# deemoe404/rmcv

Measured on AMD Instinct MI355X. Metric: frames/sec (1280x1024 BGR) armour detect, higher is better.
Workload: dtype u8

## Files before the change

rmcv_amd/csrc/contours_device.h:

```cpp
#pragma once
#include <stddef.h>
#include <stdlib.h>
#include <string.h>

#include "rmcv_internal.h"
#include "wave_detect.h"

namespace rmcv {

__device__ __forceinline__ uint64_t ld_l2(const uint64_t* p)
{
    return __hip_atomic_load(p, __ATOMIC_RELAXED, __HIP_MEMORY_SCOPE_AGENT);
}
__device__ __forceinline__ unsigned long long ld_l2(const unsigned long long* p)
{
    return __hip_atomic_load(p, __ATOMIC_RELAXED, __HIP_MEMORY_SCOPE_AGENT);
}

__device__ __forceinline__ uint64_t win_load(const uint32_t* plane32, int prow, int y, int xb)
{
    const uint32_t* p = plane32 + ((int64_t)(y + 1) * prow + 1) * 2 + (xb >> 5);
    uint64_t v;
    __builtin_memcpy(&v, p, 8);
    return v;
// ... 135 lines not shown
            const int L = __ffsll((long long)m) - 1;
            const int x0 = __shfl(found, L), y0 = band * 64 + L;
            if (lane < L) done = true;
            int len = 0, ymax = y0;
            if (lane == 0) {
                const int room = (nc < max_contours && np < max_points) ? (max_points - np) : 0;
                len = trace_border(t, x0, y0, pts + np, room, &ymax);
                if (nc < max_contours) { cs[nc] = np; cl[nc] = len; }
                __builtin_amdgcn_fence(__ATOMIC_RELEASE, "workgroup");
            }
            len = __shfl(len, 0);
            ymax = __shfl(ymax, 0);
            if (nc >= max_contours) st |= RMCV_FRAME_OVF_CONTOURS;
            if (np + len > max_points) { st |= RMCV_FRAME_OVF_POINTS; }
            nc++;
            np = (np + len > max_points) ? max_points : np + len;
            if (lane == L) { xmin = x0 + 1; dirty = true; }
            else if (lane > L && y <= ymax) dirty = true;
        }
    }
    *nc_out = nc < max_contours ? nc : max_contours;
    *np_out = np;
    *st_out = st;
}

__device__ __forceinline__ int dir_dx(int s) { return (s == 0 || s == 1 || s == 7) ? 1 : ((s >= 3 && s <= 5) ? -1 : 0); }
__device__ __forceinline__ int dir_dy(int s) { return (s >= 1 && s <= 3) ? -1 : ((s >= 5) ? 1 : 0); }

struct LabelStore {
    const uint32_t* rowmask;
    const uint16_t* rowbase;
    unsigned long long* lab;
    unsigned long long* neg;
    __device__ __forceinline__ int slot(int y, int k) const { return rowbase[y] + __popc(rowmask[y] & ((1u << k) - 1u)); }
};

#ifndef RMCV_KEPT_CAP
#define RMCV_KEPT_CAP 512
#endif
static constexpr int KEPT_CAP = RMCV_KEPT_CAP;
#ifndef RMCV_SLOT_CAP
#define RMCV_SLOT_CAP 1664
#endif
static constexpr int SLOT_CAP = RMCV_SLOT_CAP;
#ifndef RMCV_CT_THREADS_MAX
#define RMCV_CT_THREADS_MAX 512
#endif
static constexpr int CT_THREADS_MAX = RMCV_CT_THREADS_MAX;
static constexpr int MULTI_CAP = 32;
#ifndef RMCV_NN_CAP
#define RMCV_NN_CAP VISIT_CAP
#endif
static constexpr int NN_CAP = RMCV_NN_CAP;
static_assert(NN_CAP <= VISIT_CAP, "the visits' global scratch (Bufs::visit_xy) is VISIT_CAP entries per frame");
#ifndef RMCV_MID_PAD
#define RMCV_MID_PAD 0
#endif
#ifndef RMCV_CT_MAXH
#define RMCV_CT_MAXH 2048
#endif
static constexpr int CT_MAXH = RMCV_CT_MAXH;

struct ContoursLds {
    unsigned long long lab[SLOT_CAP], neg[SLOT_CAP];
    uint16_t nbase[SLOT_CAP], spos[SLOT_CAP];
    uint32_t kkey[KEPT_CAP];
    int32_t koff[KEPT_CAP], klen[KEPT_CAP];
    uint8_t kacc[KEPT_CAP];
    uint32_t multi[MULTI_CAP];
#if RMCV_MID_PAD > 0
    unsigned long long mid_pad[RMCV_MID_PAD / 8];
#endif
    int scan[CT_THREADS_MAX];
    uint32_t ringtab[256];
    uint32_t w_off[KEPT_CAP], w_cnt[KEPT_CAP];
    uint16_t n_a[NN_CAP], n_b[NN_CAP], n_d[NN_CAP];
    int nnodes, nkept, cursor, flags, nrows, nslots, nelig, lit[3];
    int nmulti;
    int revoked;
    int wnext;
    int sink[64];
};
static_assert(offsetof(ContoursLds, scan) >= (CT_THREADS_MAX / 64) * 3840, "the fused tail's wave-private rows (sizeof(WaveLds) = 3840 each) overlay dead tables only");
static_assert(offsetof(ContoursLds, scan) % 8 == 0 && offsetof(ContoursLds, w_off) % 8 == 0, "alignment");
static constexpr int MID_LDS_WORDS = (int)(offsetof(ContoursLds, scan) / 4);

struct RowTabs {
    uint32_t* rowmask;
    uint16_t* rows;
    uint16_t* rowbase;
};
__host__ __device__ static inline int lds_rows_cap(int h) { const int r = (h + 63) & ~63; return r < CT_MAXH ? r : CT_MAXH; }
__host__ __device__ static inline size_t lds_bytes(int h) { return sizeof(ContoursLds) + (size_t)lds_rows_cap(h) * 8; }
__device__ __forceinline__ RowTabs row_tabs(void* smem, int rows_cap)
{
    RowTabs R;
    R.rowmask = reinterpret_cast<uint32_t*>(reinterpret_cast<unsigned char*>(smem) + sizeof(ContoursLds));
    R.rows = reinterpret_cast<uint16_t*>(R.rowmask + rows_cap);
    R.rowbase = R.rows + rows_cap;
    return R;
}

constexpr uint32_t ring_entry(int ring)
{
    uint32_t backs[4] = {0, 0, 0, 0}, nexts[4] = {0, 0, 0, 0}, negs[4] = {0, 0, 0, 0};
    int cnt = 0, west0 = 0;
    if (ring == 0) {
        cnt = 1;
        west0 = 1;
        negs[0] = 1;
    } else {
        int wa = -1;
        for (int b = 0; b < 8; b++) {
            if (!((ring >> b) & 1)) continue;
            int d = (b + 1) & 7, axis = 0, west = 0, len = 0;
            while (!((ring >> d) & 1)) {
                axis |= !(d & 1);
                west |= d == 4;
                d = (d + 1) & 7;
                len++;
            }
            if (!len || !axis) continue;
            if (cnt < 4) {
                backs[cnt] = (uint32_t)b;
                nexts[cnt] = (uint32_t)d;
                negs[cnt] = ((unsigned)(d - 1) < (unsigned)b) ? 1u : 0u;
                if (west) wa = cnt;
            }
            cnt++;
        }
        if (wa > 0 && wa < 4) {
            uint32_t t = backs[0]; backs[0] = backs[wa]; backs[wa] = t;
            t = nexts[0]; nexts[0] = nexts[wa]; nexts[wa] = t;
            t = negs[0]; negs[0] = negs[wa]; negs[wa] = t;
        }
        west0 = wa >= 0;
    }
    uint32_t e = (uint32_t)(cnt > 7 ? 7 : cnt);
    for (int a = 0; a < 4; a++) e |= (backs[a] << (3 + 3 * a)) | (nexts[a] << (15 + 3 * a)) | (negs[a] << (28 + a));
    e |= (uint32_t)west0 << 27;
    return e;
}
struct RingTab {
    uint32_t v[256];
    constexpr RingTab() : v()
    {
        for (int r = 0; r < 256; r++) v[r] = ring_entry(r);
    }
};
static __device__ const RingTab RINGTAB = RingTab();

__device__ __forceinline__ uint32_t ring_of(int b, uint64_t ul, uint64_t uc, uint64_t ur, uint64_t ml, uint64_t mc, uint64_t mr,
                                            uint64_t dl, uint64_t dc, uint64_t dr)
{
    auto three = [&](uint64_t l, uint64_t c, uint64_t r) -> uint32_t {
        if (b == 0) return (uint32_t)(l >> 63) | ((uint32_t)(c & 3ull) << 1);
        if (b == 63) return (uint32_t)(c >> 62) | ((uint32_t)(r & 1ull) << 2);
        return (uint32_t)(c >> (b - 1)) & 7u;
    };
    const uint32_t u = three(ul, uc, ur), m = three(ml, mc, mr), d = three(dl, dc, dr);
    return ((m >> 2) & 1u) | (((u >> 2) & 1u) << 1) | (((u >> 1) & 1u) << 2) | ((u & 1u) << 3) | ((m & 1u) << 4) | ((d & 1u) << 5) |
           (((d >> 1) & 1u) << 6) | (((d >> 2) & 1u) << 7);
}

__device__ __forceinline__ void visit_masks(uint64_t ul, uint64_t uc, uint64_t ur, uint64_t ml, uint64_t mc, uint64_t mr, uint64_t dl,
                                            uint64_t dc, uint64_t dr, uint64_t* B, uint64_t* E2, uint64_t* E3, uint64_t* E4)
// ... 1055 lines not shown
```

rmcv_amd/csrc/k_contours_kernel.inc:

```
#define CT_THREADS KC_THREADS
#ifndef RMCV_KC_ATTR
#define RMCV_KC_ATTR
#endif
__global__ __launch_bounds__(CT_THREADS) RMCV_KC_ATTR void KC_KERNEL(const uint64_t* __restrict__ bits, const uint32_t* __restrict__ rowmasks,
                                                        int rm_pitch, uint64_t* lab, uint64_t* neg, int w, int h, int ww, int prow,
                                                        int64_t plane_pitch, rmcv_point* points, int32_t* cont_start,
                                                        int32_t* cont_len, int32_t* n_contours, int32_t* n_points,
                                                        int32_t* status, int max_contours, int max_points, int force_literal,
                                                        int32_t* __restrict__ elig, int32_t* __restrict__ n_elig,
                                                        int32_t* __restrict__ slot_kind, SparseTail X, uint32_t* __restrict__ visit_xy,
                                                        uint8_t* __restrict__ mid_base, int64_t mid_stride, int mid_slot_cap, SparseSched Q, int rows_cap)
{
    extern __shared__ unsigned long long smem_raw[];
#ifndef RMCV_KC_PRIO
#define RMCV_KC_PRIO 3
#endif
    __builtin_amdgcn_s_setprio(RMCV_KC_PRIO);
    ContoursLds& S = *reinterpret_cast<ContoursLds*>(smem_raw);
    const RowTabs RT = row_tabs(smem_raw, rows_cap);
    const int tid = threadIdx.x, lane = tid & 63, wave = tid >> 6;
    enum { FL_COMPLEX = 1, FL_MID = 2 };
    const int f = Q.order ? Q.order[blockIdx.x] : (int)blockIdx.x;
#ifdef RMCV_PROFILE_HANDOVER
    const long long th0_ = wall_clock64(), th1_ = th0_;
// ... 153 lines not shown
        if (tid == 0) S.flags = FL_COMPLEX;
        __syncthreads();
    }
    const bool literal = (S.flags & FL_COMPLEX) != 0;
    const bool complex = S.flags != 0;

    if (complex) {
        if (literal) {
        if (wave == 0) {
            int nc, np, st;
            literal_frame(lane, F, LAB, NEG, h, ww, prow, pts, cs, cl, max_contours, max_points,
                          summarised ? RT.rowmask : nullptr, &nc, &np, &st);
            if (lane == 0) { S.lit[0] = nc; S.lit[1] = np; S.lit[2] = st | RMCV_FRAME_SLOW_PATH; }
        }
        __threadfence();
        __syncthreads();
        for (int y = tid; y < h; y += CT_THREADS) {
            const int64_t base = (int64_t)(y + 1) * prow + 1;
            const uint32_t occ = summarised ? RT.rowmask[y] : ~0u;
            for (int k = 0; k < ww; k++)
                if ((k >= 32 || ((occ >> k) & 1u)) && F[base + k]) { LAB[base + k] = 0; NEG[base + k] = 0; }
        }
        }
        {
            const int nc = S.lit[0];
            int32_t* el = elig + (int64_t)f * max_contours;
            for (int k = tid; k < nc; k += CT_THREADS) {
                if (cl[k] >= 6) el[atomicAdd(&S.nelig, 1)] = k;
                else slot_kind[(int64_t)f * max_contours + (nc - 1 - k)] = 0;
            }
        }
        __syncthreads();
        if (tid == 0) {
            n_contours[f] = S.lit[0];
            n_points[f] = S.lit[1];
            n_elig[f] = S.nelig;
            status[f] = S.lit[2];
        }
    } else {
    STAMP();
#ifdef RMCV_PROFILE
    if (tid == 0 && (f == 0 || f == 100))
        printf("[f%d] rows=%d slots=%d nodes=%d kept=%d pts=%d | tables %.1f cycles %.1f V %.1f us\n", f, nrows, S.nslots, S.nnodes,
               nkept, S.cursor, (t_[1] - t_[0]) / 100.0, (t_[2] - t_[1]) / 100.0, (t_[3] - t_[2]) / 100.0);
#endif
    for (int e = tid; e < nkept; e += CT_THREADS) {
        const uint32_t key = S.kkey[e];
        int rank = 0;
        for (int j = 0; j < nkept; j++) rank += S.kkey[j] < key;
        cs[rank] = S.koff[e];
        cl[rank] = S.klen[e];
        if (S.klen[e] >= 6) {
            const int pos = atomicAdd(&S.nelig, 1);
            elig[(int64_t)f * max_contours + pos] = rank;
            S.n_d[pos] = (uint16_t)rank;
            S.w_off[pos] = (uint32_t)S.koff[e];
            S.w_cnt[pos] = (uint32_t)S.klen[e];
        } else slot_kind[(int64_t)f * max_contours + (nkept - 1 - rank)] = 0;
    }
    __syncthreads();
    if (tid == 0) {
        n_contours[f] = nkept;
        n_points[f] = S.cursor;
        n_elig[f] = S.nelig;
        status[f] = 0;
    }
    }
#if defined(RMCV_PROFILE) || defined(RMCV_PROFILE_HANDOVER)
    const long long tt0_ = wall_clock64();
#endif
    if (!X.fused) return;
    __syncthreads();
    const int nc = complex ? S.lit[0] : S.nkept;
    const int ne_all = S.nelig;
    const int ne_cap = !complex ? NN_CAP : (nc > 65535 ? 0 : 1024);
    const int ne = ne_all > ne_cap ? ne_cap : ne_all;
    const int32_t* el = elig + (int64_t)f * max_contours;
    uint16_t* const w_len = S.n_b;
    uint16_t* const w_idx = S.n_d;
    uint16_t* const w_sorted = S.n_a;
    const uint32_t* const w_off = S.w_off;
    const uint32_t* const w_cnt = S.w_cnt;
    static_assert(KEPT_CAP <= NN_CAP, "the work list fits the node tables");
    for (int e = tid; e < ne; e += CT_THREADS) {
        int len;
        if (complex) {
            const int k = el[e];
            len = cl[k];
            w_idx[e] = (uint16_t)k;
        } else len = (int)w_cnt[e];
        w_len[e] = (uint16_t)(len > 65535 ? 65535 : len);
    }
    if (tid == 0) S.wnext = 0;
    __syncthreads();
    for (int e = tid; e < ne; e += CT_THREADS) {
        const int len = w_len[e];
        int rank = 0;
        for (int j = 0; j < ne; j++) rank += (w_len[j] > len) || (w_len[j] == len && j < e);
        w_sorted[rank] = (uint16_t)e;
    }
    __syncthreads();
    {
        static_assert(offsetof(ContoursLds, n_a) >= (CT_THREADS_MAX / 64) * sizeof(WaveLds), "the work list must outlive the tables");
        static_assert(offsetof(ContoursLds, w_off) >= (CT_THREADS_MAX / 64) * sizeof(WaveLds), "... and so must its LDS copies of starts / lengths");
        WaveLds& L = reinterpret_cast<WaveLds*>(smem_raw)[wave];
        for (;;) {
            const int got = atomicAdd(lane == 0 ? &S.wnext : &S.sink[lane], lane == 0 ? 1 : 0);
            const int e = __shfl(got, 0);
            if (e >= ne_all) break;
            if (!complex) {
                const int pos = w_sorted[e];
                fit_contour_slot_at(f, (int)w_idx[pos], nc, pts, (int)w_off[pos], (int)w_cnt[pos], max_contours, max_points, X.G, slot_kind,
                                    X.slot_ell, L, lane);
            } else {
                const int k = e < ne ? (int)w_idx[w_sorted[e]] : el[e];
                fit_contour_slot(f, k, nc, pts, cs, cl, max_contours, max_points, X.G, slot_kind, X.slot_ell, L, lane);
            }
        }
    }
    __syncthreads();
#if defined(RMCV_PROFILE) || defined(RMCV_PROFILE_HANDOVER)
    const long long tt1_ = wall_clock64();
#endif
    if (wave == 0) {
        const FitTail& T = X.T;
        const int enemy = tail_enemy(T, f);
        const int np = blob_compact_frame(f, lane, slot_kind, X.slot_ell, nc, max_contours, enemy, T.blobs, T.blob_src, T.ellipses,
                                          T.neg_idx, T.n_blobs, T.n_neg, T.status, T.max_blobs);
        if (T.do_pairs) {
            __threadfence_block();
            armours_frame(f, lane, T.blobs, np, T.max_blobs, T.angle_diff_max, T.shear_max, T.length_ratio_max, enemy, T.armours,
                          T.n_armours, T.status, T.max_armours, T.ov);
        }
    }
#ifdef RMCV_PROFILE
    __syncthreads();
    if (tid == 0 && blockIdx.x < 2) printf("[tail b%d] eligible %d of %d contours: fits %.1f us, compaction + pairing %.1f us\n", (int)blockIdx.x, ne_all, nc, (tt1_ - tt0_) / 100.0, (wall_clock64() - tt1_) / 100.0);
#endif
#ifdef RMCV_PROFILE_HANDOVER
    __syncthreads();
    if (tid == 0)
        printf("[sp] %d %lld %lld %lld | %.1f %.1f %.1f %.1f %.1f | elig %d\n", f, th0_, th1_, (long long)wall_clock64(), (t_[1] - t_[0]) / 100.0,
               (t_[2] - t_[1]) / 100.0, (tt0_ - t_[2]) / 100.0, (tt1_ - tt0_) / 100.0, (wall_clock64() - tt1_) / 100.0, ne_all);
#endif
#ifndef KC_NO_CLASSIFY
    if (X.C.enabled) {
        __threadfence_block();
        __syncthreads();
        constexpr int NW = CT_THREADS / 64;
        static_assert((CT_THREADS_MAX / 64) * sizeof(WaveLds) + NW * (NFEAT * sizeof(float) + 32 * sizeof(double)) <= sizeof(ContoursLds), "feature rows fit");
        unsigned char* base = reinterpret_cast<unsigned char*>(smem_raw) + (CT_THREADS_MAX / 64) * sizeof(WaveLds);
        double* sums = reinterpret_cast<double*>(base) + wave * 32;
        float* feat = reinterpret_cast<float*>(base + NW * 32 * sizeof(double)) + wave * NFEAT;
        int na = X.T.n_armours[f];
        if (na > X.T.max_armours) na = X.T.max_armours;
        classify_frame(f, lane, wave, NW, na, X.C, X.T.armours, X.T.max_armours, feat, sums);
    }
#endif
}

#undef CT_THREADS
```

rmcv_amd/csrc/k_detect.hip:

```cpp
#include "device_hull.h"
#include "wave_detect.h"

namespace rmcv {

static constexpr int FIT_CHUNKS = 4;
__global__ __launch_bounds__(256) void k_fit(const rmcv_point* __restrict__ points, const int32_t* __restrict__ cont_start,
                                            const int32_t* __restrict__ cont_len, const int32_t* __restrict__ n_contours,
                                            int max_contours, int max_points, float tilt_max, float ratio_lo, float ratio_hi,
                                            double area_lo, double area_hi, int32_t* __restrict__ slot_kind,
                                            rmcv_rrect* __restrict__ slot_ell, const int32_t* __restrict__ elig,
                                            const int32_t* __restrict__ n_elig, int ov)
{
    __shared__ WaveLds lds[4];
    __builtin_amdgcn_s_setprio(3);
    const int f = blockIdx.x, lane = threadIdx.x & 63, wave = threadIdx.x >> 6;
    WaveLds& L = lds[wave];
    const int n = n_contours[f];
    const rmcv_point* pts = points + (int64_t)f * max_points;
    const int32_t* cs = cont_start + (int64_t)f * max_contours;
    const int32_t* cl = cont_len + (int64_t)f * max_contours;
    const int ne = n_elig[f];
    const FitGates G = {tilt_max, ratio_lo, ratio_hi, area_lo, area_hi, ov};
    for (int e = blockIdx.y * 4 + wave; e < ne; e += 4 * gridDim.y)
        fit_contour_slot(f, elig[(int64_t)f * max_contours + e], n, pts, cs, cl, max_contours, max_points, G, slot_kind, slot_ell, L, lane);
}

struct MatchArgs {
    float min_ratio, max_ratio, tilt_angle, min_area, max_area;
    int fit_ellipse, mode;
    int ov;
    int wcap, hcap, ccap;
    int pass;
    const uint8_t* frames;
    int64_t frame_pitch;
    int stride;
    const rmcv_point* win_eff;
};

static constexpr int MATCH_CHUNKS = 16;
static constexpr int MATCH_DEFERRED = 0x100;
__global__ __launch_bounds__(64) void k_match(const rmcv_point* __restrict__ points, const int32_t* __restrict__ cont_start,
                                             const int32_t* __restrict__ cont_len, const int32_t* __restrict__ n_contours,
                                             int max_contours, int max_points, MatchArgs A, int32_t* __restrict__ slot_kind,
                                             rmcv_rrect* __restrict__ slot_ell, const int32_t* __restrict__ elig,
                                             const int32_t* __restrict__ n_elig, int32_t* __restrict__ status)
{
    extern __shared__ unsigned long long match_smem[];
    __builtin_amdgcn_s_setprio(3);
    const int f = blockIdx.x, lane = threadIdx.x;
    WaveLds& L = *reinterpret_cast<WaveLds*>(match_smem);
    HullLds H;
    hull_lds_carve(reinterpret_cast<unsigned char*>(match_smem) + sizeof(WaveLds), A.wcap, A.hcap, A.ccap, H);
    const bool final_pass = A.pass == 1 || A.mode == 1;
    const int n = n_contours[f];
    const rmcv_point* pts = points + (int64_t)f * max_points;
    const int32_t* cs = cont_start + (int64_t)f * max_contours;
    const int32_t* cl = cont_len + (int64_t)f * max_contours;
    const int ne = A.mode == 1 ? n : n_elig[f];
    for (int e = blockIdx.y; e < ne; e += gridDim.y) {
        const int k = A.mode == 1 ? e : elig[(int64_t)f * max_contours + e];
        const int c = n - 1 - k;
        const int start = cs[k], len = cl[k];
        if (A.pass == 1 && slot_kind[(int64_t)f * max_contours + c] != MATCH_DEFERRED) continue;
        int word = 0;
        rmcv_rrect box = {0, 0, 0, 0, 0};
        if (len >= 1 && start + len <= max_points && (A.mode == 1 || len >= 6)) {
            const rmcv_point* cp = pts + start;
            double a00 = 0;
            long long sx = 0, sy = 0;
            int minx = INT_MAX, maxx = INT_MIN, miny = INT_MAX, maxy = INT_MIN;
            for (int i = lane; i < len; i += 64) {
                const rmcv_point p = cp[i], q = cp[i == 0 ? len - 1 : i - 1];
                a00 += (double)(float)q.x * (float)p.y - (double)(float)q.y * (float)p.x;
                sx += p.x;
                sy += p.y;
                minx = p.x < minx ? p.x : minx;
                maxx = p.x > maxx ? p.x : maxx;
                miny = p.y < miny ? p.y : miny;
                maxy = p.y > maxy ? p.y : maxy;
            }
            a00 = wave_sum_f64(a00);
            sx = wave_sum_i64(sx);
            sy = wave_sum_i64(sy);
            for (int d = 32; d >= 1; d >>= 1) {
                const int a = __shfl_xor(minx, d), b = __shfl_xor(maxx, d), cc = __shfl_xor(miny, d), dd = __shfl_xor(maxy, d);
                minx = a < minx ? a : minx;
                maxx = b > maxx ? b : maxx;
                miny = cc < miny ? cc : miny;
                maxy = dd > maxy ? dd : maxy;
            }
            const int W = maxx - minx + 1, Hh = maxy - miny + 1;
            const double area = dabs(a00 * 0.5);
            int ovf = 0;
            if (minx < 0 || miny < 0 || W > A.wcap || maxy >= HULL_MAX_DIM || len > (1 << 20)) ovf = 1;
            if (A.mode == 1) {
                if (!ovf) min_area_rect_wave(cp, len, minx, W, H, lane, &box, &ovf);
                word = 1;
                if (ovf && lane == 0) atomicOr(&status[f], RMCV_FRAME_HULL);
            } else if (!(area < A.min_area || area > A.max_area)) {
                rmcv_rrect ellipse;
                fit_ellipse_wave(cp, len, sx, sy, L, lane, &ellipse);
                if (A.fit_ellipse) {
                    box = ellipse;
                    ovf = 0;
                } else if (!ovf) {
                    min_area_rect_wave(cp, len, minx, W, H, lane, &box, &ovf);
                }
                if (ovf) {
                    word = final_pass ? 0 : MATCH_DEFERRED;
                    if (final_pass && lane == 0) atomicOr(&status[f], RMCV_FRAME_HULL);
                } else {
                    const float mx = box.w > box.h ? box.w : box.h, mn = box.w < box.h ? box.w : box.h;
                    const float ratio = mx / mn;
                    bool ok = !(ratio > A.max_ratio || ratio < A.min_ratio);
                    const float angle = ellipse.angle > 90 ? ellipse.angle - 90 : ellipse.angle + 90;
                    if (abs_ov(angle - 90, A.ov) > A.tilt_angle) ok = false;
                    if (ok) {
                        int camp = RMCV_CAMP_NEUTRAL;
                        if (A.frames)
                            camp = camp_from_mean_wave(A.frames + (int64_t)f * A.frame_pitch + frame_origin_offset(A.win_eff, f, A.stride), A.stride, minx, miny, W, Hh, lane);
                        word = 1 | ((camp + 2) << 4);
                    }
                }
            }
        }
        if (lane == 0) {
            slot_kind[(int64_t)f * max_contours + c] = word;
            slot_ell[(int64_t)f * max_contours + c] = box;
        }
    }
}


__global__ __launch_bounds__(64) void k_armours(const rmcv_lightblob* __restrict__ blobs, const int32_t* __restrict__ n_blobs,
                                               int max_blobs, float angle_diff_max, float shear_max,
                                               float length_ratio_max, int enemy, rmcv_armour* __restrict__ armours,
                                               int32_t* __restrict__ n_armours, int32_t* __restrict__ status, int max_armours, int ov,
                                               const int32_t* __restrict__ enemy_tab )
{
    if (enemy_tab) enemy = enemy_tab[blockIdx.x];
    armours_frame(blockIdx.x, threadIdx.x, blobs, n_blobs[blockIdx.x], max_blobs, angle_diff_max, shear_max, length_ratio_max, enemy,
                  armours, n_armours, status, max_armours, ov);
}

__global__ __launch_bounds__(64) void k_pairs(const int32_t* __restrict__ slot_kind, const rmcv_rrect* __restrict__ slot_ell,
                                             const int32_t* __restrict__ n_contours, int max_contours, FitTail T)
{
    const int f = blockIdx.x, lane = threadIdx.x;
    __builtin_amdgcn_s_setprio(3);
    const int enemy = tail_enemy(T, f);
    const int np = blob_compact_frame(f, lane, slot_kind, slot_ell, n_contours[f], max_contours, enemy, T.blobs, T.blob_src,
                                      T.ellipses, T.neg_idx, T.n_blobs, T.n_neg, T.status, T.max_blobs);
    if (T.do_pairs) {
            __threadfence_block();
        armours_frame(f, lane, T.blobs, np, T.max_blobs, T.angle_diff_max, T.shear_max, T.length_ratio_max, enemy, T.armours,
                      T.n_armours, T.status, T.max_armours, T.ov);
    }
}

static constexpr int COMPACT_FRAMES = 16;
__global__ __launch_bounds__(256) void k_compact_armours(const rmcv_armour* __restrict__ armours,
                                                        const int32_t* __restrict__ n_armours, int n_frames, int max_armours,
                                                        rmcv_armour* __restrict__ out, int cap, int32_t* __restrict__ frame_offs,
                                                        const int32_t* __restrict__ status, int32_t* __restrict__ status_or,
                                                        uint8_t* __restrict__ host_rec, int host_head, const int32_t* __restrict__ n_points)
{
    int32_t* const h_offs = reinterpret_cast<int32_t*>(host_rec);
    rmcv_armour* const h_out = reinterpret_cast<rmcv_armour*>(host_rec + host_head);
    __shared__ int s_part[256];
    __shared__ int s_base, s_st, s_mid;
    __shared__ unsigned long long s_pts;
    __shared__ int s_off[COMPACT_FRAMES], s_cnt[COMPACT_FRAMES];
    const int tid = threadIdx.x, lane = tid & 63, wave = tid >> 6;
    const int f_begin = blockIdx.x * COMPACT_FRAMES;
    if (tid == 0) { s_base = 0; s_st = 0; s_mid = 0; s_pts = 0; }
    __syncthreads();
    for (int f0 = 0; f0 < n_frames; f0 += 256) {
        const int f = f0 + tid;
        const int c = f < n_frames ? n_armours[f] : 0;
        if (status_or && blockIdx.x == 0 && f < n_frames) {
            const int st = status[f];
            if (st) { atomicOr(&s_st, st); if (st & RMCV_FRAME_MID_PATH) atomicAdd(&s_mid, 1); }
            atomicAdd(&s_pts, (unsigned long long)(n_points[f] > 0 ? n_points[f] : 0));
        }
// ... 154 lines not shown
```

rmcv_amd/csrc/wave_detect.h:

```cpp
#pragma once
#include "device_classify.h"
#include "device_fit.h"
#include "rmcv_internal.h"

namespace rmcv {

__device__ __forceinline__ int lanes_below(uint64_t m, int lane) { return __popcll(m & ((1ull << lane) - 1)); }

struct WaveLds {
    double rows[64][6];
    double terms[64];
    double dm[32];
};

__device__ __forceinline__ double wave_sum_f64(double v)
{
    for (int d = 32; d >= 1; d >>= 1) v += __shfl_xor(v, d);
    return v;
}
__device__ __forceinline__ long long wave_sum_i64(long long v)
{
    for (int d = 32; d >= 1; d >>= 1) v += __shfl_xor(v, d);
    return v;
}

template <typename F>
__device__ __forceinline__ double seq_sum_terms(int n, int lane, WaveLds& L, F term)
{
    double s = 0;
    for (int base = 0; base < n; base += 64) {
        const int i = base + lane;
        const double t = i < n ? term(i) : 0.0;
        const int m = n - base < 64 ? n - base : 64;
        if (m == 64) {
#pragma unroll
            for (int j = 0; j < 64; j++) s += lane_get(t, j);
        } else {
            for (int j = 0; j < m; j++) s += lane_get(t, j);
        }
    }
    return s;
}

template <typename F0, typename F1>
__device__ __forceinline__ void seq_sum_terms2(int n, int lane, F0 term0, F1 term1, double* s0_, double* s1_)
{
    double s0 = 0, s1 = 0;
    for (int base = 0; base < n; base += 64) {
        const int i = base + lane;
        const double t0 = i < n ? term0(i) : 0.0, t1 = i < n ? term1(i) : 0.0;
        const int m = n - base < 64 ? n - base : 64;
        if (m == 64) {
#pragma unroll
            for (int j = 0; j < 64; j++) { s0 += lane_get(t0, j); s1 += lane_get(t1, j); }
        } else {
            for (int j = 0; j < m; j++) { s0 += lane_get(t0, j); s1 += lane_get(t1, j); }
        }
    }
    *s0_ = s0;
    *s1_ = s1;
}

template <int NR, typename F>
__device__ __forceinline__ double seq_sum_products_two(int n, int lane, WaveLds& L, int ns, int la, int lb, F make_row )
{
    double acc = 0;
    const int half = lane >> 5, l5 = lane & 31;
    for (int base = 0; base < n; base += 32) {
        const int i = base + l5;
        if (i < n) {
            double r[NR];
            make_row(i, half, r);
#pragma unroll
            for (int k = 0; k < NR; k++) L.rows[lane][k] = r[k];
        }
        __builtin_amdgcn_wave_barrier();
        const int m = n - base < 32 ? n - base : 32;
        if (l5 < ns) {
            const int r0 = half * 32;
#pragma unroll 8
            for (int j = 0; j < m; j++) acc += L.rows[r0 + j][la] * L.rows[r0 + j][lb];
        }
        __builtin_amdgcn_wave_barrier();
    }
    return acc;
}

template <int NR, typename F>
__device__ __forceinline__ double seq_sum_products(int n, int lane, WaveLds& L, int ns, int la, int lb, double konst, F make_row)
{
    double acc = 0;
    for (int base = 0; base < n; base += 64) {
        const int i = base + lane;
        if (i < n) {
            double r[NR];
// ... 23 lines not shown
    constexpr int NT = K * (K + 1) / 2, NS = NT + K;
    double acc[NS];
#pragma unroll
    for (int e = 0; e < NS; e++) acc[e] = 0.0;
#pragma unroll 1
    for (int i = lane; i < n; i += 64) {
        double row[K];
        make_row(i, row);
        int e = 0;
#pragma unroll
        for (int a = 0; a < K; a++)
#pragma unroll
            for (int b = a; b < K; b++, e++) acc[e] += row[a] * row[b];
#pragma unroll
        for (int a = 0; a < K; a++) acc[NT + a] += row[a] * konst;
    }
    for (int d = 32; d >= 1; d >>= 1) {
        double o[NS];
#pragma unroll
        for (int e = 0; e < NS; e++) o[e] = __shfl_xor(acc[e], d);
#pragma unroll
        for (int e = 0; e < NS; e++) acc[e] += o[e];
    }
#pragma unroll
    for (int e = 0; e < NS; e++) out[e] = acc[e];
}

__device__ __forceinline__ void tri_index(int e, int k, int* a, int* b)
{
    int r = 0, rem = e;
    while (r < k && rem >= k - r) { rem -= k - r; r++; }
    *a = r;
    *b = r + rem;
}

template <int K, typename F>
__device__ __forceinline__ void normal_refine(NormalFac& Fac, int n, int lane, double bconst, double* x , F make_row)
{
    LaneVec xv(lane);
#pragma unroll
    for (int a = 0; a < K; a++) xv.reg = lane == a ? x[a] : xv.reg;
    for (int step = 0; step < 2; step++) {
        double xs[K];
#pragma unroll
        for (int a = 0; a < K; a++) xs[a] = xv.get(a);
        double acc[K];
#pragma unroll
        for (int a = 0; a < K; a++) acc[a] = 0.0;
#pragma unroll 1
        for (int i = lane; i < n; i += 64) {
            double row[K];
            make_row(i, row);
            double t = row[0] * xs[0];
#pragma unroll
            for (int b = 1; b < K; b++) t += row[b] * xs[b];
            const double r = bconst - t;
#pragma unroll
            for (int a = 0; a < K; a++) acc[a] += row[a] * r;
        }
        for (int d = 32; d >= 1; d >>= 1) {
            double o[K];
#pragma unroll
            for (int a = 0; a < K; a++) o[a] = __shfl_xor(acc[a], d);
#pragma unroll
            for (int a = 0; a < K; a++) acc[a] += o[a];
        }
        LaneVec h(lane);
#pragma unroll
        for (int a = 0; a < K; a++) h.reg = lane == a ? acc[a] : h.reg;
        double dx[5];
        normal_apply<K>(Fac, h, dx, lane);
#pragma unroll
        for (int a = 0; a < K; a++) xv.reg = lane == a ? xs[a] + dx[a] : xv.reg;
    }
#pragma unroll
    for (int a = 0; a < K; a++) x[a] = xv.get(a);
}

#ifdef RMCV_PROFILE_FITS
#define FSTAMP(k) do { if (prof) prof[k] = wall_clock64(); } while (0)
#else
#define FSTAMP(k) do {} while (0)
#endif
__device__ inline int fit_ellipse_wave(const rmcv_point* __restrict__ pts, int n, long long sumx, long long sumy, WaveLds& L, int lane,
                                rmcv_rrect* box, long long* prof = nullptr)
{
    FSTAMP(0);
    bool g_have = false;
    double g_s = 0;
    {
        const double cx = (double)sumx / n, cy = (double)sumy / n;
        g_have = sumx < (1ll << 24) && sumy < (1ll << 24);
        const float gcx = (float)sumx / (float)n, gcy = (float)sumy / (float)n;
        double s;
        if (g_have) {
            seq_sum_terms2(n, lane,
                           [&](int i) { return dabs((float)pts[i].x - cx) + dabs((float)pts[i].y - cy); },
                           [&](int i) { const float px = (float)pts[i].x - gcx, py = (float)pts[i].y - gcy; return dabs((double)px) + dabs((double)py); },
                           &s, &g_s);
        } else {
            s = seq_sum_terms(n, lane, L, [&](int i) { return dabs((float)pts[i].x - cx) + dabs((float)pts[i].y - cy); });
        }
        const double scale = 100.0 / (s > FLT_EPSILON ? s : (double)FLT_EPSILON);
        FSTAMP(1);
        int la = 0, lb = 0;
        tri_index((lane & 31) < 21 ? (lane & 31) : 0, 6, &la, &lb);
        double DM[6][6], TM[3][3], M[3][3], Ts = 0;
        const float eps1 = (float)(s / (n * 2) * 1e-2);
        const double acc = seq_sum_products_two<6>(n, lane, L, 21, la, lb, [&](int i, int set, double* r) {
            float ox, oy;
            get_ofs(i, set ? eps1 : 0.0f, &ox, &oy);
            const double px = (((float)pts[i].x + ox) - cx) * scale, py = (((float)pts[i].y + oy) - cy) * scale;
            r[0] = px * px; r[1] = px * py; r[2] = py * py; r[3] = px; r[4] = py; r[5] = 1.0;
        });
        const double inv_n = 1.0 / n;
        if ((lane & 31) < 21) (lane < 32 ? L.dm : L.terms)[lane & 31] = acc * inv_n;
        __builtin_amdgcn_wave_barrier();
        int iter;
        {
            const double* src = lane < 32 ? L.dm : L.terms;
            {
                int e = 0;
#pragma unroll
                for (int a = 0; a < 6; a++)
#pragma unroll
                    for (int b = a; b < 6; b++, e++) DM[a][b] = DM[b][a] = src[e];
            }
            const double det = direct_reduce(DM, TM, &Ts, M);
            const double det0 = lane_get(det, 0), det1 = lane_get(det, 32);
            iter = dabs(det0) > 1.0e-10 ? 0 : (dabs(det1) > 1.0e-10 ? 1 : 2);
            const int sel = iter == 1 ? 32 : 0;
#pragma unroll
            for (int a = 0; a < 3; a++)
#pragma unroll
                for (int b = 0; b < 3; b++) {
                    TM[a][b] = lane_get(TM[a][b], sel);
                    M[a][b] = lane_get(M[a][b], sel);
                }
            Ts = lane_get(Ts, sel);
        }
        __builtin_amdgcn_wave_barrier();
        FSTAMP(2);
        if (iter < 2) {
            direct_finish(M, TM, Ts, scale, cx, cy, box, lane);
            FSTAMP(3);
            if (is_good_box(box)) return 0;
        }
        FSTAMP(3);
    }
    {
        float cx, cy;
        if (sumx < (1ll << 24) && sumy < (1ll << 24)) {
            cx = (float)sumx;
            cy = (float)sumy;
        } else {
            cx = 0;
            cy = 0;
            for (int i = 0; i < n; i++) { cx += (float)pts[i].x; cy += (float)pts[i].y; }
        }
        cx /= (float)n;
        cy /= (float)n;
        const double s = g_have ? g_s : seq_sum_terms(n, lane, L, [&](int i) {
            const float px = (float)pts[i].x - cx, py = (float)pts[i].y - cy;
            return dabs((double)px) + dabs((double)py);
        });
        const double scale = 100.0 / (s > FLT_EPSILON ? s : (double)FLT_EPSILON);
        FSTAMP(8);
// ... 9 lines not shown
                const float fx = ((float)pts[i].x + ox) - cx, fy = ((float)pts[i].y + oy) - cy;
                const double px = fx * scale, py = fy * scale;
                r[0] = -px * px; r[1] = -py * py; r[2] = -px * py; r[3] = px; r[4] = py;
            };
            {
                double sums[20];
                par_sum_products<5>(n, lane, 10000.0, sums, row5);
#pragma unroll
                for (int e = 0; e < 20; e++)
                    if (lane == e) L.dm[e] = sums[e];
            }
            __builtin_amdgcn_wave_barrier();
            LaneVec G(lane), g(lane);
            {
                const int a = lane / 5, b = lane - 5 * a;
                const int lo = a < b ? a : b, hi = a < b ? b : a;
                const int e = lo * 5 - lo * (lo - 1) / 2 + (hi - lo);
                G.reg = lane < 25 ? L.dm[e] : 0.0;
                g.reg = lane < 5 ? L.dm[15 + lane] : 0.0;
            }
            __builtin_amdgcn_wave_barrier();
            FSTAMP(9);
            NormalFac Fac(lane);
            double wmax, wmin;
            normal_factor<5>(G, Fac, &wmax, &wmin);
            FSTAMP(10);
            if (iter == 0 && wmax * FLT_EPSILON > wmin) {
                eps = (float)(s / (n * 2) * 1e-3);
                continue;
            }
            normal_apply<5>(Fac, g, gfp, lane);
            FSTAMP(11);
            normal_refine<5>(Fac, n, lane, 10000.0, gfp, row5);
            break;
        }
        FSTAMP(4);
        general_centre(gfp, rp);
        if (lane < 6) tri_index(lane, 3, &la, &lb);
        else { la = lane < 9 ? lane - 6 : 0; lb = -1; }
        const double r0 = rp[0], r1 = rp[1];
        auto row3 = [&](int i, double* r) {
            float ox = 0, oy = 0;
            if (eps != 0.0f) get_ofs(i, eps, &ox, &oy);
            const float fx = ((float)pts[i].x + ox) - cx, fy = ((float)pts[i].y + oy) - cy;
            const double px = fx * scale, py = fy * scale;
            r[0] = (px - r0) * (px - r0); r[1] = (py - r1) * (py - r1); r[2] = (px - r0) * (py - r1);
        };
        {
            double sums[9];
            par_sum_products<3>(n, lane, 1.0, sums, row3);
#pragma unroll
            for (int e = 0; e < 9; e++)
                if (lane == e) L.dm[e] = sums[e];
        }
        __builtin_amdgcn_wave_barrier();
        LaneVec G(lane), g(lane);
        {
            const int a = lane / 3, b = lane - 3 * a;
            const int lo = a < b ? a : b, hi = a < b ? b : a;
            const int e = lo * 3 - lo * (lo - 1) / 2 + (hi - lo);
            G.reg = lane < 9 ? L.dm[e] : 0.0;
            g.reg = lane < 3 ? L.dm[6 + lane] : 0.0;
        }
        __builtin_amdgcn_wave_barrier();
        FSTAMP(5);
        NormalFac Fac(lane);
        double wmax3, wmin3;
        normal_factor<3>(G, Fac, &wmax3, &wmin3);
        normal_apply<3>(Fac, g, gfp, lane);
        FSTAMP(12);
        normal_refine<3>(Fac, n, lane, 1.0, gfp, row3);
        FSTAMP(13);
        general_finish(gfp, rp, scale, cx, cy, box);
        FSTAMP(6);
    }
    return 1;
}

struct FitGates {
    float tilt_max, ratio_lo, ratio_hi;
    double area_lo, area_hi;
    int ov;
};
__device__ inline void fit_contour_slot_at(int f, int k, int n, const rmcv_point* __restrict__ pts, int start, int len, int max_contours,
                                           int max_points, const FitGates& G, int32_t* __restrict__ slot_kind,
                                           rmcv_rrect* __restrict__ slot_ell, WaveLds& L, int lane)
{
    const int c = n - 1 - k;
    int kind = 0;
    rmcv_rrect ell = {0, 0, 0, 0, 0};
    if (len >= 6 && start + len <= max_points) {
        const rmcv_point* cp = pts + start;
        double a00 = 0;
        long long sx = 0, sy = 0;
        for (int i = lane; i < len; i += 64) {
            const rmcv_point p = cp[i], q = cp[i == 0 ? len - 1 : i - 1];
            a00 += (double)(float)q.x * (float)p.y - (double)(float)q.y * (float)p.x;
            sx += p.x;
            sy += p.y;
        }
        a00 = wave_sum_f64(a00);
        sx = wave_sum_i64(sx);
        sy = wave_sum_i64(sy);
        const double area = dabs(a00 * 0.5);
        if (area >= G.area_lo && area <= G.area_hi) {
#ifdef RMCV_PROFILE_FITS
            long long pr[16] = {0, 0, 0, 0, 0, 0, 0, 0, 0, 0, 0, 0, 0, 0, 0, 0};
            const int path = fit_ellipse_wave(cp, len, sx, sy, L, lane, &ell, pr);
            if (lane == 0 && ((f == 0 && len > 150) || (path == 1 && f < 64)))
                printf("[fit f%d c%d n=%d path=%d] s %.1f moments+reduce %.1f finish %.1f | gen: s %.1f sums20 %.1f jacobi5 %.1f apply %.1f refine5 %.1f | "
                       "centre+sums9 %.1f jacobi3+apply %.1f refine3 %.1f finish %.1f us\n", f, c, len, path, (pr[1] - pr[0]) / 100.0,
                       (pr[2] - pr[1]) / 100.0, (pr[3] - pr[2]) / 100.0, (pr[8] - pr[3]) / 100.0, (pr[9] - pr[8]) / 100.0, (pr[10] - pr[9]) / 100.0,
                       (pr[11] - pr[10]) / 100.0, (pr[4] - pr[11]) / 100.0, (pr[5] - pr[4]) / 100.0, (pr[12] - pr[5]) / 100.0,
                       (pr[13] - pr[12]) / 100.0, (pr[6] - pr[13]) / 100.0);
#else
            fit_ellipse_wave(cp, len, sx, sy, L, lane, &ell);
#endif
            bool negative = false;
            const float mx = ell.w > ell.h ? ell.w : ell.h, mn = ell.w < ell.h ? ell.w : ell.h;
            const float ratio = mx / mn;
            if (!(ratio >= G.ratio_lo && ratio <= G.ratio_hi)) negative = true;
            const float angle = ell.angle > 90 ? ell.angle - 90 : ell.angle + 90;
            if (abs_ov(angle - 90, G.ov) > G.tilt_max) negative = true;
            kind = negative ? 2 : 1;
        }
    }
    if (lane == 0) {
        slot_kind[(int64_t)f * max_contours + c] = kind;
        slot_ell[(int64_t)f * max_contours + c] = ell;
    }
}

__device__ inline void fit_contour_slot(int f, int k, int n, const rmcv_point* __restrict__ pts, const int32_t* __restrict__ cs,
                                        const int32_t* __restrict__ cl, int max_contours, int max_points, const FitGates& G,
                                        int32_t* __restrict__ slot_kind, rmcv_rrect* __restrict__ slot_ell, WaveLds& L, int lane)
{
    fit_contour_slot_at(f, k, n, pts, cs[k], cl[k], max_contours, max_points, G, slot_kind, slot_ell, L, lane);
}

struct FitTail {
    rmcv_lightblob* blobs;
    int32_t* blob_src;
    rmcv_rrect* ellipses;
    int32_t* neg_idx;
    int32_t* n_blobs;
    int32_t* n_neg;
    int32_t* status;
    rmcv_armour* armours;
    int32_t* n_armours;
    int max_blobs, max_armours, enemy, do_pairs;
    float angle_diff_max, shear_max, length_ratio_max;
    int ov;
    const int32_t* enemy_tab;
};
__device__ __forceinline__ int tail_enemy(const FitTail& T, int f)
{
    return T.enemy_tab ? T.enemy_tab[f] : T.enemy;
}

__device__ inline int blob_compact_frame(int f, int lane, const int32_t* slot_kind, const rmcv_rrect* slot_ell, int n, int max_contours,
                                  int enemy, rmcv_lightblob* blobs, int32_t* blob_src, rmcv_rrect* ellipses, int32_t* neg_idx,
                                  int32_t* n_blobs, int32_t* n_neg, int32_t* status, int max_blobs)
{
    rmcv_lightblob* ob = blobs + (int64_t)f * max_blobs;
    int32_t* osrc = blob_src + (int64_t)f * max_blobs;
    rmcv_rrect* oell = ellipses + (int64_t)f * max_blobs;
    int32_t* oneg = neg_idx + (int64_t)f * max_contours;
    int np = 0, nn = 0;
    for (int base = 0; base < n; base += 64) {
        const int c = base + lane;
        const int word = c < n ? slot_kind[(int64_t)f * max_contours + c] : 0;
        const int kind = word & 15, camp_code = word >> 4;
        const uint64_t mp = __ballot(kind == 1), mn_ = __ballot(kind == 2);
        if (kind == 1) {
            const int o = np + lanes_below(mp, lane);
            if (o < max_blobs) {
                const rmcv_rrect ell = slot_ell[(int64_t)f * max_contours + c];
                make_lightblob(&ell, camp_code ? camp_code - 2 : enemy, &ob[o]);
                osrc[o] = c;
                oell[o] = ell;
            }
        } else if (kind == 2) {
            oneg[nn + lanes_below(mn_, lane)] = c;
        }
        np += __popcll(mp);
        nn += __popcll(mn_);
    }
    if (np > max_blobs) {
        if (lane == 0) atomicOr(&status[f], RMCV_FRAME_OVF_BLOBS);
        np = max_blobs;
    }
    if (lane == 0) {
        n_blobs[f] = np;
        n_neg[f] = nn;
    }
    return np;
}

__device__ __forceinline__ bool pair_ok(const rmcv_lightblob& a, const rmcv_lightblob& b, float angle_diff_max,
                                        float shear_max, float length_ratio_max, int ov)
{
    const float angle_difference = abs_ov(a.angle - b.angle, ov);
    if (angle_difference > angle_diff_max) return false;
    const float y = abs_ov(a.center[1] - b.center[1], ov);
    const float x = abs_ov(a.center[0] - b.center[0], ov);
    const float rect_angle = atan2_deg_ov(y, x, ov);
    const float shear_i = abs_ov(a.angle > 90 ? abs_ov(a.angle - rect_angle, ov) - 90 : abs_ov(180 - a.angle - rect_angle, ov) - 90, ov);
    const float shear_j = abs_ov(b.angle > 90 ? abs_ov(b.angle - rect_angle, ov) - 90 : abs_ov(180 - b.angle - rect_angle, ov) - 90, ov);
    if (shear_i > shear_max || shear_j > shear_max) return false;
    const float hi = a.size[1], hj = b.size[1];
    const float mn = hi < hj ? hi : hj, mx = hi < hj ? hj : hi;
    if (mn / mx < length_ratio_max) return false;
    if (abs_ov(a.center[1] - b.center[1], ov) > (a.size[1] + b.size[1]) / 2) return false;
    if (abs_ov(a.center[0] - b.center[0], ov) > (a.size[1] + b.size[1]) * 2) return false;
    return true;
}

__device__ inline void armours_frame(int f, int lane, const rmcv_lightblob* blobs, int n, int max_blobs, float angle_diff_max,
                                     float shear_max, float length_ratio_max, int enemy, rmcv_armour* armours, int32_t* n_armours,
                                     int32_t* status, int max_armours, int ov)
{
    const rmcv_lightblob* lb = blobs + (int64_t)f * max_blobs;
    rmcv_armour* out = armours + (int64_t)f * max_armours;
    int na = 0;
    if (n >= 2) {
        const int total = n * (n - 1) / 2;
        int i = 0, rem = lane;
        while (i < n - 1 && rem >= n - 1 - i) { rem -= n - 1 - i; i++; }
        for (int base = 0; base < total; base += 64) {
            const int j = i + 1 + rem;
            bool ok = false;
            rmcv_lightblob a, b;
            if (base + lane < total) {
                a = lb[i];
                b = lb[j];
                ok = a.target == enemy && b.target == enemy && pair_ok(a, b, angle_diff_max, shear_max, length_ratio_max, ov);
            }
            const uint64_t m = __ballot(ok);
            if (ok) {
                const int o = na + lanes_below(m, lane);
                if (o < max_armours) {
                    make_armour(&a, &b, &out[o], ov);
                    out[o].blob_i = i;
                    out[o].blob_j = j;
                }
            }
            na += __popcll(m);
            rem += 64;
            while (i < n - 1 && rem >= n - 1 - i) { rem -= n - 1 - i; i++; }
        }
    }
    if (lane == 0) {
        if (na > max_armours) {
            atomicOr(&status[f], RMCV_FRAME_OVF_ARMOURS);
            na = max_armours;
        }
        n_armours[f] = na;
    }
}

struct SparseTail {
    int fused;
    FitGates G;
    rmcv_rrect* slot_ell;
    FitTail T;
    ClassifyArgs C;
};

hipError_t launch_contours_w4(const Geom& g, const Bufs& b, const Limits& lim, const SparseTail& X, int flags, const SparseSched& Q, int grid,
                              SparseLds lds, hipStream_t s);
hipError_t launch_contours_lean(const Geom& g, const Bufs& b, const Limits& lim, const SparseTail& X, int flags, const SparseSched& Q, int grid, SparseLds lds,
                                hipStream_t s);

}
```

Baseline: 1.197 million.

## Stage fit points, slot results and kept blobs in LDS for the fused tail

The ellipse-fit path now copies each contour's points into a per-wave LDS cache as packed 16-bit coordinates, so repeated passes over the points read LDS instead of global memory. Slot kinds and ellipses are also written to LDS for the simple path, and blob compaction reads them from there. Up to 64 compacted light blobs are kept in LDS for the pairing stage, which lets it skip the block fence in the common case. This adds LDS overlay aliasing and extra copy work per contour, and it depends on the static layout assertions holding.

Result: no change. 1.207 million (median of 6 runs) (+0.9%).

```diff
diff --git a/rmcv_amd/csrc/contours_device.h b/rmcv_amd/csrc/contours_device.h
--- a/rmcv_amd/csrc/contours_device.h
+++ b/rmcv_amd/csrc/contours_device.h
@@ -241,6 +241,7 @@
     int sink[64];
 };
 static_assert(offsetof(ContoursLds, scan) >= (CT_THREADS_MAX / 64) * 3840, "the fused tail's wave-private rows (sizeof(WaveLds) = 3840 each) overlay dead tables only");
+static_assert(offsetof(ContoursLds, scan) >= (CT_THREADS_MAX / 64) * (3840 + 256 * 4), "... and so do the fits' point caches behind them (FIT_PT_CACHE = 256 packed points each)");
 static_assert(offsetof(ContoursLds, scan) % 8 == 0 && offsetof(ContoursLds, w_off) % 8 == 0, "alignment");
 static constexpr int MID_LDS_WORDS = (int)(offsetof(ContoursLds, scan) / 4);
 
diff --git a/rmcv_amd/csrc/k_contours_kernel.inc b/rmcv_amd/csrc/k_contours_kernel.inc
--- a/rmcv_amd/csrc/k_contours_kernel.inc
+++ b/rmcv_amd/csrc/k_contours_kernel.inc
@@ -259,6 +259,15 @@
     const uint32_t* const w_off = S.w_off;
     const uint32_t* const w_cnt = S.w_cnt;
     static_assert(KEPT_CAP <= NN_CAP, "the work list fits the node tables");
+    static_assert((NN_CAP - KEPT_CAP) * sizeof(uint16_t) + NN_CAP * sizeof(uint16_t) >= KEPT_CAP * (sizeof(int32_t) + sizeof(rmcv_rrect)) &&
+                  offsetof(ContoursLds, n_b) == offsetof(ContoursLds, n_a) + NN_CAP * sizeof(uint16_t) && offsetof(ContoursLds, n_a) % 4 == 0 &&
+                  (NN_CAP - KEPT_CAP) * sizeof(uint16_t) >= KEPT_CAP * sizeof(int32_t),
+                  "the slots' LDS copy fits behind the work list, its kinds in front of n_b");
+    const bool hand_lds = !complex && nc <= KEPT_CAP;
+    int32_t* const hand_kind = reinterpret_cast<int32_t*>(S.n_a + KEPT_CAP);
+    const SlotHand hand = {hand_lds, hand_kind, reinterpret_cast<rmcv_rrect*>(hand_kind + KEPT_CAP)};
+    if (hand_lds)
+        for (int c = tid; c < nc; c += CT_THREADS) hand_kind[c] = 0;
     for (int e = tid; e < ne; e += CT_THREADS) {
         int len;
         if (complex) {
@@ -281,6 +290,9 @@
         static_assert(offsetof(ContoursLds, n_a) >= (CT_THREADS_MAX / 64) * sizeof(WaveLds), "the work list must outlive the tables");
         static_assert(offsetof(ContoursLds, w_off) >= (CT_THREADS_MAX / 64) * sizeof(WaveLds), "... and so must its LDS copies of starts / lengths");
         WaveLds& L = reinterpret_cast<WaveLds*>(smem_raw)[wave];
+        static_assert((CT_THREADS_MAX / 64) * sizeof(WaveLds) + (CT_THREADS / 64) * FIT_PT_CACHE * sizeof(uint32_t) <= offsetof(ContoursLds, scan),
+                      "the point caches overlay dead tables only");
+        uint32_t* const pcache = reinterpret_cast<uint32_t*>(reinterpret_cast<unsigned char*>(smem_raw) + (CT_THREADS_MAX / 64) * sizeof(WaveLds)) + wave * FIT_PT_CACHE;
         for (;;) {
             const int got = atomicAdd(lane == 0 ? &S.wnext : &S.sink[lane], lane == 0 ? 1 : 0);
             const int e = __shfl(got, 0);
@@ -288,10 +300,10 @@
             if (!complex) {
                 const int pos = w_sorted[e];
                 fit_contour_slot_at(f, (int)w_idx[pos], nc, pts, (int)w_off[pos], (int)w_cnt[pos], max_contours, max_points, X.G, slot_kind,
-                                    X.slot_ell, L, lane);
+                                    X.slot_ell, L, lane, pcache, hand);
             } else {
                 const int k = e < ne ? (int)w_idx[w_sorted[e]] : el[e];
-                fit_contour_slot(f, k, nc, pts, cs, cl, max_contours, max_points, X.G, slot_kind, X.slot_ell, L, lane);
+                fit_contour_slot_at(f, k, nc, pts, cs[k], cl[k], max_contours, max_points, X.G, slot_kind, X.slot_ell, L, lane, pcache, SlotHand{false, hand.kind, hand.ell});
             }
         }
     }
@@ -302,12 +314,16 @@
     if (wave == 0) {
         const FitTail& T = X.T;
         const int enemy = tail_enemy(T, f);
+        constexpr int BLOB_KEEP = 64;
+        static_assert(BLOB_KEEP * sizeof(rmcv_lightblob) <= sizeof(WaveLds), "the kept blobs fit wavefront 0's rows");
+        rmcv_lightblob* const keep = reinterpret_cast<rmcv_lightblob*>(smem_raw);
         const int np = blob_compact_frame(f, lane, slot_kind, X.slot_ell, nc, max_contours, enemy, T.blobs, T.blob_src, T.ellipses,
-                                          T.neg_idx, T.n_blobs, T.n_neg, T.status, T.max_blobs);
+                                          T.neg_idx, T.n_blobs, T.n_neg, T.status, T.max_blobs, hand, keep, BLOB_KEEP);
         if (T.do_pairs) {
-            __threadfence_block();
+            if (np > BLOB_KEEP) __threadfence_block();
+            __builtin_amdgcn_wave_barrier();
             armours_frame(f, lane, T.blobs, np, T.max_blobs, T.angle_diff_max, T.shear_max, T.length_ratio_max, enemy, T.armours,
-                          T.n_armours, T.status, T.max_armours, T.ov);
+                          T.n_armours, T.status, T.max_armours, T.ov, keep, np < BLOB_KEEP ? np : BLOB_KEEP);
         }
     }
 #ifdef RMCV_PROFILE
diff --git a/rmcv_amd/csrc/k_detect.hip b/rmcv_amd/csrc/k_detect.hip
--- a/rmcv_amd/csrc/k_detect.hip
+++ b/rmcv_amd/csrc/k_detect.hip
@@ -12,6 +12,7 @@
                                             const int32_t* __restrict__ n_elig, int ov)
 {
     __shared__ WaveLds lds[4];
+    __shared__ uint32_t pcache[4][FIT_PT_CACHE];
     __builtin_amdgcn_s_setprio(3);
     const int f = blockIdx.x, lane = threadIdx.x & 63, wave = threadIdx.x >> 6;
     WaveLds& L = lds[wave];
@@ -22,7 +23,7 @@
     const int ne = n_elig[f];
     const FitGates G = {tilt_max, ratio_lo, ratio_hi, area_lo, area_hi, ov};
     for (int e = blockIdx.y * 4 + wave; e < ne; e += 4 * gridDim.y)
-        fit_contour_slot(f, elig[(int64_t)f * max_contours + e], n, pts, cs, cl, max_contours, max_points, G, slot_kind, slot_ell, L, lane);
+        fit_contour_slot(f, elig[(int64_t)f * max_contours + e], n, pts, cs, cl, max_contours, max_points, G, slot_kind, slot_ell, L, lane, pcache[wave]);
 }
 
 struct MatchArgs {
@@ -99,7 +100,7 @@
                 if (ovf && lane == 0) atomicOr(&status[f], RMCV_FRAME_HULL);
             } else if (!(area < A.min_area || area > A.max_area)) {
                 rmcv_rrect ellipse;
-                fit_ellipse_wave(cp, len, sx, sy, L, lane, &ellipse);
+                fit_ellipse_wave(FitPts{cp, nullptr, 0}, len, sx, sy, L, lane, &ellipse);
                 if (A.fit_ellipse) {
                     box = ellipse;
                     ovf = 0;
diff --git a/rmcv_amd/csrc/wave_detect.h b/rmcv_amd/csrc/wave_detect.h
--- a/rmcv_amd/csrc/wave_detect.h
+++ b/rmcv_amd/csrc/wave_detect.h
@@ -11,6 +11,31 @@
     double rows[64][6];
     double terms[64];
     double dm[32];
+};
+
+template <typename T>
+__device__ __forceinline__ T lds_read(const T* p)
+{
+#if defined(__HIP_DEVICE_COMPILE__)
+    return *(const __attribute__((address_space(3))) T*)p;
+#else
+    return *p;
+#endif
+}
+static constexpr int FIT_PT_CACHE = 256;
+static_assert(FIT_PT_CACHE % 64 == 0 && FIT_PT_CACHE >= 256, "whole chunks; the plain stream's longest contour has 224 points");
+struct FitPts {
+    const rmcv_point* g;
+    const uint32_t* c;
+    int cap;
+    __device__ __forceinline__ rmcv_point operator[](int i) const
+    {
+        if (i < cap) {
+            const uint32_t v = lds_read(&c[i]);
+            return rmcv_point{(int32_t)(v & 0xFFFFu), (int32_t)(v >> 16)};
+        }
+        return g[i];
+    }
 };
 
 __device__ __forceinline__ double wave_sum_f64(double v)
@@ -200,7 +225,7 @@
 #else
 #define FSTAMP(k) do {} while (0)
 #endif
-__device__ inline int fit_ellipse_wave(const rmcv_point* __restrict__ pts, int n, long long sumx, long long sumy, WaveLds& L, int lane,
+__device__ inline int fit_ellipse_wave(const FitPts& pts, int n, long long sumx, long long sumy, WaveLds& L, int lane,
                                 rmcv_rrect* box, long long* prof = nullptr)
 {
     FSTAMP(0);
@@ -376,15 +401,42 @@
     double area_lo, area_hi;
     int ov;
 };
+struct SlotHand {
+    bool on;
+    int32_t* kind;
+    rmcv_rrect* ell;
+};
 __device__ inline void fit_contour_slot_at(int f, int k, int n, const rmcv_point* __restrict__ pts, int start, int len, int max_contours,
                                            int max_points, const FitGates& G, int32_t* __restrict__ slot_kind,
-                                           rmcv_rrect* __restrict__ slot_ell, WaveLds& L, int lane)
+                                           rmcv_rrect* __restrict__ slot_ell, WaveLds& L, int lane, uint32_t* pcache = nullptr,
+                                           SlotHand hand = SlotHand{false, nullptr, nullptr})
 {
     const int c = n - 1 - k;
     int kind = 0;
     rmcv_rrect ell = {0, 0, 0, 0, 0};
     if (len >= 6 && start + len <= max_points) {
-        const rmcv_point* cp = pts + start;
+        FitPts cp = {pts + start, pcache, 0};
+        if (pcache) {
+            constexpr int NCH = FIT_PT_CACHE / 64;
+            rmcv_point v[NCH];
+            bool fits16 = true;
+#pragma unroll
+            for (int u = 0; u < NCH; u++) {
+                const int i = u * 64 + lane;
+                v[u] = i < len ? cp.g[i] : rmcv_point{0, 0};
+            }
+#pragma unroll
+            for (int u = 0; u < NCH; u++) fits16 = fits16 && (((uint32_t)v[u].x | (uint32_t)v[u].y) >> 16) == 0;
+            if (__all(fits16)) {
+#pragma unroll
+                for (int u = 0; u < NCH; u++) {
+                    const int i = u * 64 + lane;
+                    if (i < len) pcache[i] = (uint32_t)v[u].x | ((uint32_t)v[u].y << 16);
+                }
+                cp.cap = FIT_PT_CACHE;
+            }
+            __builtin_amdgcn_wave_barrier();
+        }
         double a00 = 0;
         long long sx = 0, sy = 0;
         for (int i = lane; i < len; i += 64) {
@@ -422,14 +474,19 @@
     if (lane == 0) {
         slot_kind[(int64_t)f * max_contours + c] = kind;
         slot_ell[(int64_t)f * max_contours + c] = ell;
+        if (hand.on) {
+            hand.kind[c] = kind;
+            hand.ell[c] = ell;
+        }
     }
 }
 
 __device__ inline void fit_contour_slot(int f, int k, int n, const rmcv_point* __restrict__ pts, const int32_t* __restrict__ cs,
                                         const int32_t* __restrict__ cl, int max_contours, int max_points, const FitGates& G,
-                                        int32_t* __restrict__ slot_kind, rmcv_rrect* __restrict__ slot_ell, WaveLds& L, int lane)
-{
-    fit_contour_slot_at(f, k, n, pts, cs[k], cl[k], max_contours, max_points, G, slot_kind, slot_ell, L, lane);
+                                        int32_t* __restrict__ slot_kind, rmcv_rrect* __restrict__ slot_ell, WaveLds& L, int lane,
+                                        uint32_t* pcache = nullptr)
+{
+    fit_contour_slot_at(f, k, n, pts, cs[k], cl[k], max_contours, max_points, G, slot_kind, slot_ell, L, lane, pcache);
 }
 
 struct FitTail {
@@ -454,7 +511,8 @@
 
 __device__ inline int blob_compact_frame(int f, int lane, const int32_t* slot_kind, const rmcv_rrect* slot_ell, int n, int max_contours,
                                   int enemy, rmcv_lightblob* blobs, int32_t* blob_src, rmcv_rrect* ellipses, int32_t* neg_idx,
-                                  int32_t* n_blobs, int32_t* n_neg, int32_t* status, int max_blobs)
+                                  int32_t* n_blobs, int32_t* n_neg, int32_t* status, int max_blobs,
+                                  SlotHand hand = SlotHand{false, nullptr, nullptr}, rmcv_lightblob* keep = nullptr, int keep_cap = 0)
 {
     rmcv_lightblob* ob = blobs + (int64_t)f * max_blobs;
     int32_t* osrc = blob_src + (int64_t)f * max_blobs;
@@ -463,14 +521,22 @@
     int np = 0, nn = 0;
     for (int base = 0; base < n; base += 64) {
         const int c = base + lane;
-        const int word = c < n ? slot_kind[(int64_t)f * max_contours + c] : 0;
+        const int word = c < n ? (hand.on ? lds_read(&hand.kind[c]) : slot_kind[(int64_t)f * max_contours + c]) : 0;
         const int kind = word & 15, camp_code = word >> 4;
         const uint64_t mp = __ballot(kind == 1), mn_ = __ballot(kind == 2);
         if (kind == 1) {
             const int o = np + lanes_below(mp, lane);
             if (o < max_blobs) {
-                const rmcv_rrect ell = slot_ell[(int64_t)f * max_contours + c];
-                make_lightblob(&ell, camp_code ? camp_code - 2 : enemy, &ob[o]);
+                rmcv_rrect ell;
+                if (hand.on) {
+                    const float* e = &hand.ell[c].cx;
+                    ell = rmcv_rrect{lds_read(e), lds_read(e + 1), lds_read(e + 2), lds_read(e + 3), lds_read(e + 4)};
+                }
+                else ell = slot_ell[(int64_t)f * max_contours + c];
+                rmcv_lightblob b;
+                make_lightblob(&ell, camp_code ? camp_code - 2 : enemy, &b);
+                ob[o] = b;
+                if (o < keep_cap) keep[o] = b;
                 osrc[o] = c;
                 oell[o] = ell;
             }
@@ -512,7 +578,7 @@
 
 __device__ inline void armours_frame(int f, int lane, const rmcv_lightblob* blobs, int n, int max_blobs, float angle_diff_max,
                                      float shear_max, float length_ratio_max, int enemy, rmcv_armour* armours, int32_t* n_armours,
-                                     int32_t* status, int max_armours, int ov)
+                                     int32_t* status, int max_armours, int ov, const rmcv_lightblob* kept = nullptr, int n_kept = 0)
 {
     const rmcv_lightblob* lb = blobs + (int64_t)f * max_blobs;
     rmcv_armour* out = armours + (int64_t)f * max_armours;
@@ -526,8 +592,10 @@
             bool ok = false;
             rmcv_lightblob a, b;
             if (base + lane < total) {
-                a = lb[i];
-                b = lb[j];
+                if (i < n_kept) a = lds_read(&kept[i]);
+                else a = lb[i];
+                if (j < n_kept) b = lds_read(&kept[j]);
+                else b = lb[j];
                 ok = a.target == enemy && b.target == enemy && pair_ok(a, b, angle_diff_max, shear_max, length_ratio_max, ov);
             }
             const uint64_t m = __ballot(ok);
```
